# MiraPurkrabek/ProbPose_code

Measured on AMD Instinct MI355X. Metric: person-crops/sec @ 256x192 bs64, higher is better.
Workload: dtype f16x3; 1 GPU; ProbPose-small (ViT-S 12x384, 12 heads x 32) bs64 random 256x192 uint8 crops per GPU, flip_test=True, seeded random-init weights: preprocess -> backbone x2 passes -> ProbMapHead (heatmap branch + Sparsemax + 4 towers) -> ProbMap decode -> results in pinned host memory; crops_per_gpu=64, global_batch=64, parallelism=dp1, steps_in_flight=2

## Files before the change

probpose_code_amd/csrc/pp_api.hip:

```cpp
#include "pp_common.h"

#include <cstring>
#include <mutex>

namespace pp {

static thread_local char g_last_error[512] = "";

void set_error(const char* fmt, ...) {
    va_list ap;
    va_start(ap, fmt);
    vsnprintf(g_last_error, sizeof(g_last_error), fmt, ap);
    va_end(ap);
}

struct Option { const char* name; int value; };
static Option g_options[] = {
    {"panel", 1},
    {"conv_halo", 1},
    {"psplit_nst", 0},
    {"panel_linear_mink", 0},
    {"psplit_bf16_conv", 0},
    {"psplit_tap_inner", 1},
    {"psplit_conv_weight_major", 1},
    {"attn_dma", 1},
    {"conv_pool_split", 1},
    {"decode_wgs_per_cu", 3},
    {"linear_dma", 1},
    {"linear_loop", 1},
    {"psplit_deconv_weight_major", 0},
    {"ffn_pair", 1},
    {"psplit_tail", 1},
    {"wino_order", 8},
    {"ksplit_channels", 1},
    {"qkv_attn_deep", 1},
    {"skinny_tile", 0},
    {"qkv_attn_qsplit", 1},
    {"skinny_xcd_order", 1},
    {"ksplit9_below", 1024},
};

struct LaunchCount {
    char name[48];
    long long n;
};
static LaunchCount g_launches[96];
static int g_n_launches = 0;
static std::mutex g_launch_mutex;

void count_launch(const char* file_or_tag) {
    std::lock_guard<std::mutex> lock(g_launch_mutex);
    const char* base = file_or_tag;
    for (const char* c = file_or_tag; *c; ++c)
        if (*c == '/') base = c + 1;
    for (int i = 0; i < g_n_launches; ++i)
        if (std::strcmp(g_launches[i].name, base) == 0) {
            ++g_launches[i].n;
            return;
        }
    if (g_n_launches < (int)(sizeof(g_launches) / sizeof(g_launches[0]))) {
        std::snprintf(g_launches[g_n_launches].name, sizeof(g_launches[0].name), "%s", base);
        g_launches[g_n_launches++].n = 1;
    }
}

int option(const char* name) {
    for (const Option& o : g_options)
        if (std::strcmp(o.name, name) == 0) return o.value;
    return 0;
}

__global__ void clock_probe_kernel(unsigned long long* out, const unsigned long long* stop, unsigned long long ticks) {
    if (threadIdx.x != 0) return;
    const unsigned long long r0 = __builtin_amdgcn_s_memrealtime();
    const unsigned long long c0 = __builtin_amdgcn_s_memtime();
    unsigned long long r1 = r0;
    for (long long guard = 0; guard < (1ll << 21) && r1 - r0 < ticks; ++guard) {
        if (stop && __hip_atomic_load(stop, __ATOMIC_RELAXED, __HIP_MEMORY_SCOPE_SYSTEM) != 0) break;
        __builtin_amdgcn_s_sleep(127);
        r1 = __builtin_amdgcn_s_memrealtime();
    }
    const unsigned long long c1 = __builtin_amdgcn_s_memtime();
    r1 = __builtin_amdgcn_s_memrealtime();
    __hip_atomic_store(out + 0, c1 - c0, __ATOMIC_RELAXED, __HIP_MEMORY_SCOPE_SYSTEM);
    __hip_atomic_store(out + 1, r1 - r0, __ATOMIC_RELAXED, __HIP_MEMORY_SCOPE_SYSTEM);
}

}

extern "C" {

int pp_set_option(const char* name, int value) {
    using namespace pp;
    PP_REQUIRE(name, PP_ERR_INVALID_ARG, "pp_set_option: NULL name");
    for (Option& o : g_options)
        if (std::strcmp(o.name, name) == 0) {
            o.value = value;
            return PP_OK;
        }
    set_error("pp_set_option: unknown option '%s'", name);
    return PP_ERR_INVALID_ARG;
}

int pp_get_option(const char* name, int* value) {
    using namespace pp;
    PP_REQUIRE(name && value, PP_ERR_INVALID_ARG, "pp_get_option: NULL argument");
    for (const Option& o : g_options)
        if (std::strcmp(o.name, name) == 0) {
            *value = o.value;
            return PP_OK;
        }
    set_error("pp_get_option: unknown option '%s'", name);
    return PP_ERR_INVALID_ARG;
}

long long pp_launch_count(const char* kernel) {
    using namespace pp;
    if (!kernel) {
        set_error("pp_launch_count: NULL name");
        return 0;
    }
    std::lock_guard<std::mutex> lock(g_launch_mutex);
    for (int i = 0; i < g_n_launches; ++i)
        if (std::strcmp(g_launches[i].name, kernel) == 0) return g_launches[i].n;
    return 0;
}

int pp_reset_launch_counts(void) {
    std::lock_guard<std::mutex> lock(pp::g_launch_mutex);
    pp::g_n_launches = 0;
    return PP_OK;
}

long long pp_workspace_bytes(int buffer, int index, const pp_plan_shape* sh) {
    using namespace pp;
    if (!sh || sh->n_img <= 0 || sh->n_tokens <= 0 || sh->embed <= 0 || sh->ffn <= 0 || sh->n_keypoints <= 0 || sh->feat_h <= 0 || sh->feat_w <= 0 ||
        (sh->prec != PP_PREC_BF16 && sh->prec != PP_PREC_F32 && sh->prec != PP_PREC_F16X3)) {
        set_error("pp_workspace_bytes: bad plan shape");
        return PP_ERR_INVALID_ARG;
    }
    const long long esz = sh->prec == PP_PREC_BF16 ? 2 : 4;
    const long long M = (long long)sh->n_img * sh->n_tokens, E = sh->embed;
    auto tower_hw = [&](int j, long long& h, long long& w, long long& ph, long long& pw) {
        h = sh->feat_h;
        w = sh->feat_w;
        for (int i = 0;; ++i) {
            ph = i == 0 ? 4 : 2;
            pw = i == 0 ? 3 : 2;
            if (i == j) return;
            h /= ph;
            w /= pw;
        }
    };
    switch (buffer) {
        case PP_WS_PATCHES: return M * sh->patch_k * esz;
        case PP_WS_X: return M * E * 4;
        case PP_WS_H: case PP_WS_FEAT: case PP_WS_ATT: case PP_WS_LN2: return M * E * esz;
        case PP_WS_QKV: return M * 3 * E * esz;
        case PP_WS_FFN: return M * (long long)sh->ffn * esz;
        case PP_WS_LOGITS: return (long long)sh->n_img * sh->n_keypoints * sh->heat_h * sh->heat_w * 4;
        case PP_WS_DECONV: {
            if (index < 0 || index >= 8 || sh->deconv_channels <= 0) break;
            const long long up = 2ll << index;
            return (long long)sh->n_img * sh->feat_h * up * sh->feat_w * up * sh->deconv_channels * esz;
        }
        case PP_WS_TOWER: case PP_WS_TOWER_PARTIAL: case PP_WS_TOWER_POOLED: {
            if (index < 0 || index > 2) break;
            long long h, w, ph, pw;
            tower_hw(index, h, w, ph, pw);
            if (buffer == PP_WS_TOWER) return 4ll * sh->n_img * h * w * E * esz;
            if (buffer == PP_WS_TOWER_PARTIAL)
                return (long long)pp_conv3x3_splitk_slices(sh->prec, sh->n_img, (int)h, (int)w, sh->embed, sh->embed, 4) * 4 * sh->n_img * h * w * E * 4;
            return 4ll * sh->n_img * (h / ph) * (w / pw) * E * esz;
        }
        case PP_WS_LN_STATS: return E % 96 == 0 ? M * (E / 96) * 8 : 0;
        case PP_WS_WINOGRAD: {
            const long long n = pp_winograd_scratch_bytes(sh->n_img, sh->feat_h, sh->feat_w, sh->embed);
            return n > 0 ? n : 0;
        }
        default: break;
    }
    set_error("pp_workspace_bytes: unknown buffer %d (index %d)", buffer, index);
    return PP_ERR_INVALID_ARG;
}
// ... 58 lines not shown
```

probpose_code_amd/csrc/pp_ffn_dma.hip:

```cpp
#include "pp_common.h"
#include "pp_device.h"
#include "pp_split.h"
#include "pp_ffn_params.h"

namespace pp {
namespace ffd {

using ffs::Params;

constexpr int BM = 96, E = 384, CHUNK = 128;
constexpr int CW = 8, WAVES = 12, THREADS = WAVES * 64;
constexpr int KB = E / 32;
constexpr int G_KB = BM * 128;
constexpr int OFF_G = 0;
constexpr int OFF_RING = 4 * G_KB;
constexpr int SLOTB = 28 * 1024, NSLOT = 4;
constexpr int LDS = OFF_RING + NSLOT * SLOTB;
constexpr int X_OFF = 16 * 1024;
constexpr int NA = KB, NB = 8, STEPS = NA + NB;
constexpr int A_BLOCK = CHUNK * 128;
constexpr int B_BLOCK = (E / 2) * 128;
constexpr int B_PART = NA * A_BLOCK;
constexpr int CHUNK_BYTES = B_PART + NB * B_BLOCK;
constexpr int NPROJ = 2 * KB;
// ... 39 lines not shown

template <bool PROJ, bool PAIR>
__device__ __forceinline__ void dma_role(const Params& p, char* smem, int d, int lane, int m0, int nchunks, int c_rot) {
    char* const ring = smem + OFF_RING;
    const int x_l = lane >> 3;
    const unsigned v_w = (unsigned)lane * 16u;
    const unsigned v_x = (unsigned)(m0 + x_l) * (unsigned)(E * 4) + (unsigned)(((lane & 7) ^ x_l) << 4);

    if constexpr (PROJ) {
        auto issue_p = [&](int s) {
            if (s >= NPROJ) return;
            const __amdgpu_buffer_rsrc_t rw = buffer_rsrc(p.wproj, p.wproj_bytes);
#pragma unroll
            for (int u = 0; u < 6; ++u) {
                const int q = d + 4 * u;
                dma16(rw, ring + (s & 3) * SLOTB + q * 1024, v_w, s * B_BLOCK + q * 1024);
            }
            if ((s & 1) == 0) {
                const int kb = s >> 1;
                const __amdgpu_buffer_rsrc_t ra = buffer_rsrc(p.att, p.att_bytes);
#pragma unroll
                for (int u = 0; u < 3; ++u) {
                    const int q = d + 4 * u;
                    dma16(ra, smem + OFF_G + (kb & 3) * G_KB + q * 1024, v_x, kb * 128 + q * 8 * E * 4);
                }
            }
        };
        issue_p(0);
        issue_p(1);
        issue_p(2);
#pragma unroll
        for (int s = 0; s < NPROJ; ++s) {
            __builtin_amdgcn_sched_barrier(0);
            wait_vm_n(n_proj(s + 1) + n_proj(s + 2));
            __builtin_amdgcn_s_barrier();
            __builtin_amdgcn_sched_barrier(0);
            issue_p(s + 3);
        }
        __builtin_amdgcn_s_barrier();
        __builtin_amdgcn_s_barrier();
        __builtin_amdgcn_s_barrier();
        __builtin_amdgcn_s_barrier();
    }

    auto issue = [&](int ci, int t) {
        const bool live = ci < nchunks;
        int c = (live ? ci : 0) + c_rot;
        c = c >= nchunks ? c - nchunks : c;
        const int base = c * CHUNK_BYTES;
        const __amdgpu_buffer_rsrc_t rw = buffer_rsrc(p.wpack, live ? p.w_bytes : 0u);
        char* dst = ring + (t & 3) * SLOTB;
        if (t < NA) {
            const int kb = (ci & 1) ? NA - 1 - t : t;
#pragma unroll
            for (int u = 0; u < 4; ++u) {
                const int q = d + 4 * u;
                dma16(rw, dst + q * 1024, v_w, base + kb * A_BLOCK + q * 1024);
            }
            const __amdgpu_buffer_rsrc_t rh = buffer_rsrc(p.h, live ? p.h_bytes : 0u);
#pragma unroll
            for (int u = 0; u < 3; ++u) {
                const int q = d + 4 * u;
                dma16(rh, dst + X_OFF + q * 1024, v_x, kb * 128 + q * 8 * E * 4);
            }
        } else {
            const int sb = t - NA;
#pragma unroll
            for (int u = 0; u < 6; ++u) {
                const int q = d + 4 * u;
                dma16(rw, dst + q * 1024, v_w, base + B_PART + sb * B_BLOCK + q * 1024);
            }
        }
    };
    if constexpr (PAIR) {
        const int npairs = nchunks >> 1;
        auto issue2 = [&](int cp_, int t) {
            int cp = cp_;
            asm volatile("" : "+s"(cp));
            const bool live = cp < npairs;
            const int cpl = live ? cp : 0;
            const __amdgpu_buffer_rsrc_t rw = buffer_rsrc(p.wpack, live ? p.w_bytes : 0u);
            char* dst = ring + (t & 3) * SLOTB;
            if (t < 2 * NA) {
                int c = 2 * cpl + (t & 1) + c_rot;
                c = c >= nchunks ? c - nchunks : c;
                const int kb = (cp & 1) ? NA - 1 - (t >> 1) : (t >> 1);
#pragma unroll
                for (int u = 0; u < 4; ++u) {
                    const int q = d + 4 * u;
                    dma16(rw, dst + q * 1024, v_w, c * CHUNK_BYTES + kb * A_BLOCK + q * 1024);
                }
                if ((t & 1) == 0) {
                    const __amdgpu_buffer_rsrc_t rh = buffer_rsrc(p.h, live ? p.h_bytes : 0u);
#pragma unroll
                    for (int u = 0; u < 3; ++u) {
                        const int q = d + 4 * u;
                        dma16(rh, dst + X_OFF + q * 1024, v_x, kb * 128 + q * 8 * E * 4);
                    }
                }
            } else {
                const int which = (t - 2 * NA) >> 3, sb = (t - 2 * NA) & 7;
                int c = 2 * cpl + which + c_rot;
                c = c >= nchunks ? c - nchunks : c;
#pragma unroll
                for (int u = 0; u < 6; ++u) {
                    const int q = d + 4 * u;
                    dma16(rw, dst + q * 1024, v_w, c * CHUNK_BYTES + B_PART + sb * B_BLOCK + q * 1024);
                }
            }
        };
        constexpr int PS = 2 * STEPS;
        auto n2 = [](int t) { t %= PS; return t < 2 * NA ? ((t & 1) == 0 ? 7 : 4) : 6; };
        issue2(0, 0);
        issue2(0, 1);
        issue2(0, 2);
        for (int cp = 0; cp < npairs; ++cp) {
#pragma unroll
            for (int t = 0; t < PS; ++t) {
                __builtin_amdgcn_sched_barrier(0);
                wait_vm_n(n2(t + 1) + n2(t + 2));
                __builtin_amdgcn_s_barrier();
                __builtin_amdgcn_sched_barrier(0);
                if (t + 3 < PS) issue2(cp, t + 3); else issue2(cp + 1, t + 3 - PS);
                if (t == 2 * NA || t == 2 * NA + NB) __builtin_amdgcn_s_barrier();
            }
        }
    } else {
    issue(0, 0);
    issue(0, 1);
    issue(0, 2);
    for (int ci = 0; ci < nchunks; ++ci) {
#pragma unroll
        for (int t = 0; t < STEPS; ++t) {
            __builtin_amdgcn_sched_barrier(0);
            wait_vm_n(n_main(t + 1) + n_main(t + 2));
            __builtin_amdgcn_s_barrier();
            __builtin_amdgcn_sched_barrier(0);
            if (t + 3 < STEPS) issue(ci, t + 3); else issue(ci + 1, t + 3 - STEPS);
            if (t == NA) __builtin_amdgcn_s_barrier();
        }
    }
    }
    wait_vm<0>();
    __builtin_amdgcn_s_barrier();
    __builtin_amdgcn_s_barrier();
    __builtin_amdgcn_s_barrier();
}

#if FFD_STAMP
__device__ unsigned long long g_ffd_stamps[2][64];
#endif
struct TagF { static constexpr bool value = false; };
struct TagT { static constexpr bool value = true; };
template <bool PROJ, bool PAIR, int FOLD = 0>
__device__ __forceinline__ void compute_role(const Params& p, char* smem, int wv, int lane, int m0, int nchunks, int c_rot) {
    const int rg = wv >> 2, cg = wv & 3;
    const int f_row = lane & 15, f_kg = lane >> 4;
    auto chunk_of = [&](int i) { const int c = i + c_rot; return c >= nchunks ? c - nchunks : c; };
#if FFD_STAMP
    int n_stamp = 0;
    auto stamp = [&]() {
        if (wv == 0 && (blockIdx.x == 0 || blockIdx.x == 131)) {
            const unsigned long long t = __builtin_amdgcn_s_memtime();
            if (lane == 0 && n_stamp < 64) g_ffd_stamps[blockIdx.x == 0 ? 0 : 1][n_stamp] = t;
            ++n_stamp;
        }
    };
#else
    auto stamp = []() {};
#endif
    stamp();

    const int sw = f_row & 7;
    const int lane_hi = f_row * 128 + ((f_kg ^ sw) << 4), lane_lo = f_row * 128 + (((4 + f_kg) ^ sw) << 4);
    const int rows0 = rg * 48 + f_row;
    auto opaque_s = [](int v) { asm volatile("" : "+s"(v)); return v; };
    auto rd = [&](int lane_off, int uni, int imm) -> u32x4 { return *reinterpret_cast<const u32x4*>(smem + (lane_off + uni) + imm); };
    const int u_a = OFF_RING + cg * 32 * 128;
    const int u_b = OFF_RING + cg * 48 * 128;
    const int u_x = OFF_RING + X_OFF + rg * 48 * 128;
    const int u_g = OFF_G + rg * 48 * 128;

    f32x4 acc[3][6];
    f32x4 pacc[3][2];
    f32x4 b1v[2];
    u32x4 bgh[3], bgl[3];

    auto step_barrier = [&]() {
        __builtin_amdgcn_sched_barrier(0);
        wait_vm_lgkm<63>();
        __builtin_amdgcn_s_barrier();
        __builtin_amdgcn_sched_barrier(0);
    };
    auto b_step = [&](int slot, int half, int gbuf, bool load_g) {
        u32x4 wh[3], wl[3];
        const int ub = opaque_s(u_b + slot * SLOTB);
        const int ug = opaque_s(u_g + gbuf * G_KB);
        wh[0] = rd(lane_hi, ub, 0);
        if (load_g) bgh[0] = rd(lane_hi, ug, 0);
        wh[1] = rd(lane_hi, ub, 2048);
        wh[2] = rd(lane_hi, ub, 4096);
        if (load_g) {
            bgh[1] = rd(lane_hi, ug, 2048);
            bgh[2] = rd(lane_hi, ug, 4096);
        }
#pragma unroll
        for (int nf = 0; nf < 3; ++nf) wl[nf] = rd(lane_lo, ub, nf * 2048);
        if (load_g) {
#pragma unroll
            for (int rf = 0; rf < 3; ++rf) bgl[rf] = rd(lane_lo, ug, rf * 2048);
        }
        __builtin_amdgcn_sched_barrier(0);
#pragma unroll
        for (int rf = 0; rf < 3; ++rf)
#pragma unroll
            for (int nf = 0; nf < 3; ++nf) acc[rf][half * 3 + nf] = mma_f16(wh[nf], bgh[rf], acc[rf][half * 3 + nf]);
        __builtin_amdgcn_sched_barrier(0);
#pragma unroll
        for (int rf = 0; rf < 3; ++rf)
#pragma unroll
            for (int nf = 0; nf < 3; ++nf) acc[rf][half * 3 + nf] = mma_f16(wl[nf], bgh[rf], acc[rf][half * 3 + nf]);
        __builtin_amdgcn_sched_barrier(0);
#pragma unroll
        for (int nf = 0; nf < 3; ++nf)
#pragma unroll
            for (int rf = 0; rf < 3; ++rf) acc[rf][half * 3 + nf] = mma_f16(wh[nf], bgl[rf], acc[rf][half * 3 + nf]);
    };
    (void)b_step;
    auto layernorm_rows = [&](const float* gamma, const float* beta, float* x_dst, void* h_dst, bool store_x, auto fold_c) {
        constexpr bool FO = decltype(fold_c)::value;
        unsigned ones_ = ~0u;
        asm volatile("" : "+s"(ones_));
        const int ln_ = (int)__builtin_amdgcn_mbcnt_hi(ones_, __builtin_amdgcn_mbcnt_lo(ones_, 0u));
        const int fk_ = ln_ >> 4;
        const int rows0_ = rg * 48 + (ln_ & 15);
        auto shx = [&](float v, int m) -> float { return __builtin_bit_cast(float, __builtin_amdgcn_ds_bpermute((ln_ ^ m) << 2, __builtin_bit_cast(int, v))); };
        const unsigned row_ = (unsigned)(m0 + rows0_) * (unsigned)(E * 4);
        const unsigned v_rowx = row_ + (unsigned)fk_ * 16u;
        const unsigned v_rowh = row_ + (unsigned)fk_ * 8u;
        const unsigned v_rowh2 = row_ + (unsigned)(fk_ >> 1) * 16u + (unsigned)(fk_ & 1) * 64u;
        (void)v_rowh;
        const __amdgpu_buffer_rsrc_t rx = buffer_rsrc(x_dst, p.h_bytes);
        const __amdgpu_buffer_rsrc_t rh = buffer_rsrc(h_dst, p.h_bytes);
        float* stat = reinterpret_cast<float*>(smem + OFF_G);
        float mean[3], rstd[3];
#pragma unroll
        for (int rf = 0; rf < 3; ++rf) {
            float sm = 0.f;
#pragma unroll
            for (int cf = 0; cf < 6; ++cf) {
                const f32x4 v = acc[rf][cf];
                sm += (v[0] + v[1]) + (v[2] + v[3]);
            }
            sm += shx(sm, 16);
            sm += shx(sm, 32);
            if (fk_ == 0) stat[cg * BM + rows0_ + rf * 16] = sm;
        }
        __syncthreads();
#pragma unroll
        for (int rf = 0; rf < 3; ++rf) {
            const int r = rows0_ + rf * 16;
            mean[rf] = ((stat[r] + stat[BM + r]) + (stat[2 * BM + r] + stat[3 * BM + r])) * (1.0f / E);
            float q = 0.f;
#pragma unroll
            for (int cf = 0; cf < 6; ++cf)
#pragma unroll
                for (int k = 0; k < 4; ++k) {
                    const float dd = acc[rf][cf][k] - mean[rf];
                    q = __builtin_fmaf(dd, dd, q);
                }
            q += shx(q, 16);
            q += shx(q, 32);
            if (fk_ == 0) stat[(4 + cg) * BM + r] = q;
        }
        __syncthreads();
#if FFD_STAMP == 2
        stamp();
#endif
#pragma unroll
        for (int rf = 0; rf < 3; ++rf) {
            const int r = rows0_ + rf * 16;
            const float var = ((stat[4 * BM + r] + stat[5 * BM + r]) + (stat[6 * BM + r] + stat[7 * BM + r])) * (1.0f / E);
            rstd[rf] = 1.0f / sqrtf(var + p.eps);
            if (FO && fk_ == 0 && cg == 0 && m0 + r < p.M) {
                *reinterpret_cast<f32x2*>(p.stats_out + (size_t)(m0 + r) * 2) = f32x2{mean[rf], rstd[rf]};
            }
        }
        f32x4 gs_[6], bs_[6];
#pragma unroll
        for (int cf = 0; cf < 6; ++cf) {
            const int cb = (cf / 3) * 192 + cg * 48 + (cf % 3) * 16;
            gs_[cf] = FO ? f32x4{1.f, 1.f, 1.f, 1.f} : *reinterpret_cast<const f32x4*>(gamma + cb + fk_ * 4);
            bs_[cf] = FO ? f32x4{0.f, 0.f, 0.f, 0.f} : *reinterpret_cast<const f32x4*>(beta + cb + fk_ * 4);
        }
#pragma unroll
        for (int cf = 0; cf < 6; ++cf) {
            const int cb = (cf / 3) * 192 + cg * 48 + (cf % 3) * 16;
            const f32x4 g = gs_[cf], b = bs_[cf];
#pragma unroll
            for (int rf = 0; rf < 3; ++rf) {
                const f32x4 v = acc[rf][cf];
                float mu = mean[rf];
                const float rs = rstd[rf];
                asm("" : "+v"(mu));
                f32x4 hv = {(v[0] - mu) * rs * g[0] + b[0], (v[1] - mu) * rs * g[1] + b[1], (v[2] - mu) * rs * g[2] + b[2],
                            (v[3] - mu) * rs * g[3] + b[3]};
                if (FO) hv = f32x4{v[0] - mu, v[1] - mu, v[2] - mu, v[3] - mu};
#pragma unroll
                for (int j = 0; j < 4; ++j) { float t = hv[j]; split_pin(t); hv[j] = t; }
                if (store_x) {
                    const u32x4 vq = __builtin_bit_cast(u32x4, v);
                    store16_guarded(vq, rx, v_rowx + rf * (16 * E * 4), cb * 4);
                }
                u32x2 hu, lu;
                { unsigned h__, l__; split_pair(hv[0], hv[1], h__, l__); hu[0] = h__; lu[0] = l__; }
                { unsigned h__, l__; split_pair(hv[2], hv[3], h__, l__); hu[1] = h__; lu[1] = l__; }
                const int so = (cb >> 5) * 128 + (cb & 16) * 2;
                {
                    const auto s0 = __builtin_amdgcn_permlane16_swap(hu[0], lu[0], false, false);
                    const auto s1 = __builtin_amdgcn_permlane16_swap(hu[1], lu[1], false, false);
                    u32x4 q = {s0[0], s1[0], s0[1], s1[1]};
                    store16_guarded(q, rh, v_rowh2 + rf * (16 * E * 4), so);
                }
            }
        }
    };

    float res_mean[3] = {0.f, 0.f, 0.f};
    if constexpr ((FOLD & 1) != 0) {
#pragma unroll
        for (int rf = 0; rf < 3; ++rf) {
            const int r = m0 + rows0 + rf * 16;
            res_mean[rf] = r < p.M ? p.res_stats[(size_t)r * 2] : 0.f;
        }
    }
    const __amdgpu_buffer_rsrc_t rres = buffer_rsrc(p.residual, p.h_bytes);
    const unsigned v_rowx = (unsigned)(m0 + rows0) * (unsigned)(E * 4) + (unsigned)f_kg * 16u;
#pragma unroll
    for (int rf = 0; rf < 3; ++rf)
#pragma unroll
        for (int cf = 0; cf < 6; ++cf) {
            const int cb = (cf / 3) * 192 + cg * 48 + (cf % 3) * 16;
            if constexpr ((FOLD & 1) != 0) {
                const unsigned vsp = (unsigned)(m0 + rows0) * (unsigned)(E * 4) + (unsigned)(f_kg >> 1) * 16u + (unsigned)(f_kg & 1) * 64u;
                const u32x4 q = __builtin_bit_cast(u32x4, __builtin_amdgcn_raw_buffer_load_b128(rres, vsp + rf * (16 * E * 4), (cb >> 5) * 128 + (cb & 16) * 2, 0));
                const auto s0 = __builtin_amdgcn_permlane16_swap(q[0], q[2], false, false);
                const auto s1 = __builtin_amdgcn_permlane16_swap(q[1], q[3], false, false);
                const f16x4 hh = __builtin_bit_cast(f16x4, u32x2{s0[0], s1[0]}), ll = __builtin_bit_cast(f16x4, u32x2{s0[1], s1[1]});
                const float mu = res_mean[rf];
                acc[rf][cf] = f32x4{((float)hh[0] + (float)ll[0]) + mu, ((float)hh[1] + (float)ll[1]) + mu, ((float)hh[2] + (float)ll[2]) + mu,
                                    ((float)hh[3] + (float)ll[3]) + mu};
            } else {
                acc[rf][cf] = __builtin_bit_cast(f32x4, __builtin_amdgcn_raw_buffer_load_b128(rres, v_rowx + rf * (16 * E * 4), cb * 4, 0));
            }
        }

    stamp();
    {
        const float s_in = PROJ ? p.s_p : p.s_2;
#pragma unroll
        for (int cf = 0; cf < 6; ++cf) {
            f32x4 bv = {0.f, 0.f, 0.f, 0.f};
            if constexpr (!PROJ) bv = *reinterpret_cast<const f32x4*>(p.b2 + (cf / 3) * 192 + cg * 48 + (cf % 3) * 16 + f_kg * 4);
#pragma unroll
            for (int rf = 0; rf < 3; ++rf) acc[rf][cf] = (acc[rf][cf] + bv) * s_in;
        }
    }
    if constexpr (PROJ) {
        {
            u32x4 pwh[3], pwl[3];
            step_barrier();
            {
                const int ub = opaque_s(u_b), ug = opaque_s(u_g);
#pragma unroll
                for (int nf = 0; nf < 3; ++nf) { pwh[nf] = rd(lane_hi, ub, nf * 2048); pwl[nf] = rd(lane_lo, ub, nf * 2048); }
#pragma unroll
                for (int rf = 0; rf < 3; ++rf) { bgl[rf] = rd(lane_lo, ug, rf * 2048); bgh[rf] = rd(lane_hi, ug, rf * 2048); }
            }
#pragma unroll 1
            for (int kp = 0; kp < NPROJ / 4; ++kp) {
#pragma unroll
                for (int q = 0; q < 4; ++q) {
                    const int half = q & 1;
                    const int ub_n = opaque_s(u_b + ((q + 1) & 3) * SLOTB);
                    const int ug_n = opaque_s(u_g + ((((4 * kp + q) >> 1) + 1) & 3) * G_KB);
                    const bool nb = q < 3 || kp + 1 < NPROJ / 4;
                    const bool newg = nb && half == 1;
                    __builtin_amdgcn_sched_barrier(0);
#pragma unroll
                    for (int i = 0; i < 9; ++i) {
                        const int rf = i / 3, nf = i % 3;
                        acc[rf][half * 3 + nf] = mma_f16(pwh[nf], bgl[rf], acc[rf][half * 3 + nf]);
                        __builtin_amdgcn_sched_barrier(0);
                        if (i == 1 && nb) step_barrier();
                        if (nf == 2 && newg) bgl[rf] = rd(lane_lo, ug_n, rf * 2048);
                        __builtin_amdgcn_sched_barrier(0);
                    }
#pragma unroll
                    for (int i = 0; i < 9; ++i) {
                        const int rf = i / 3, nf = i % 3;
                        acc[rf][half * 3 + nf] = mma_f16(pwh[nf], bgh[rf], acc[rf][half * 3 + nf]);
                        __builtin_amdgcn_sched_barrier(0);
                        if (rf == 2 && nb) pwh[nf] = rd(lane_hi, ub_n, nf * 2048);
                        __builtin_amdgcn_sched_barrier(0);
                    }
#pragma unroll
                    for (int i = 0; i < 9; ++i) {
                        const int rf = i / 3, nf = i % 3;
                        acc[rf][half * 3 + nf] = mma_f16(pwl[nf], bgh[rf], acc[rf][half * 3 + nf]);
                        __builtin_amdgcn_sched_barrier(0);
                        if (nf == 2 && newg) bgh[rf] = rd(lane_hi, ug_n, rf * 2048);
                        if (rf == 2 && nb) pwl[nf] = rd(lane_lo, ub_n, nf * 2048);
                        __builtin_amdgcn_sched_barrier(0);
                    }
                }
            }
        }
#pragma unroll
        for (int cf = 0; cf < 6; ++cf) {
            const f32x4 bv = *reinterpret_cast<const f32x4*>(p.bp + (cf / 3) * 192 + cg * 48 + (cf % 3) * 16 + f_kg * 4);
#pragma unroll
            for (int rf = 0; rf < 3; ++rf) acc[rf][cf] = acc[rf][cf] * p.inv_p + bv;
        }
        stamp();
        __syncthreads();
#if FFD_STAMP == 2
        stamp();
#endif
        layernorm_rows(p.gamma2, p.beta2, nullptr, const_cast<void*>(p.h), false, TagF{});
#if FFD_STAMP == 2
        stamp();
#endif
        wait_vm_lgkm<0>();
#if FFD_STAMP == 2
        stamp();
#endif
        __syncthreads();
        stamp();
    }

    if constexpr (PROJ) {
#pragma unroll
        for (int cf = 0; cf < 6; ++cf) {
            const f32x4 bv = *reinterpret_cast<const f32x4*>(p.b2 + (cf / 3) * 192 + cg * 48 + (cf % 3) * 16 + f_kg * 4);
#pragma unroll
            for (int rf = 0; rf < 3; ++rf) acc[rf][cf] = (acc[rf][cf] + bv) * p.s_2;
        }
    }
    auto load_b1 = [&](int ci) {
        const int c = chunk_of(ci < nchunks ? ci : 0);
#pragma unroll
        for (int nf = 0; nf < 2; ++nf) b1v[nf] = *reinterpret_cast<const f32x4*>(p.b1 + c * CHUNK + cg * 32 + nf * 16 + f_kg * 4);
    };
    load_b1(0);

    auto gelu_chunk = [&](f32x4 (&pa)[3][2]) __attribute__((always_inline)) {
#pragma unroll
        for (int rf = 0; rf < 3; ++rf)
#pragma unroll
            for (int nf = 0; nf < 2; ++nf) {
                int ln_ = lane;
                asm volatile("" : "+v"(ln_));
                const int fk_ = ln_ >> 4, sw_ = ln_ & 7;
                char* gs = smem + OFF_G + cg * G_KB + (rg * 48 + (ln_ & 15) + rf * 16) * 128 + (fk_ & 1) * 8;
                const int c = 2 * nf + (fk_ >> 1);
                const int sw = sw_;
                unsigned hq[2], lq[2];
#pragma unroll
                for (int u0 = 0; u0 < 2; ++u0) {
                    const f32x2 x = f32x2{pa[rf][nf][2 * u0], pa[rf][nf][2 * u0 + 1]} * p.inv_1;
                    const f32x2 ax = __builtin_elementwise_abs(x);
                    const f32x2 d = ax * 0.23164189265f + 1.0f;
                    const f32x2 t = {__builtin_amdgcn_rcpf(d[0]), __builtin_amdgcn_rcpf(d[1])};
                    const f32x2 uu = x * 0.84932180028801904272f;
                    const f32x2 u2 = uu * uu;
                    const f32x2 e = {__builtin_amdgcn_exp2f(-u2[0]), __builtin_amdgcn_exp2f(-u2[1])};
                    f32x2 q = t * 1.061405429f + -1.453152027f;
                    q = t * q + 1.421413741f;
                    q = t * q + -0.284496736f;
                    q = t * q + 0.254829592f;
                    const f32x2 erfc_z = (t * q) * e;
                    const f32x2 ma = ax * -0.5f;
                    const f32x2 mx = x * 0.5f - ma;
                    f32x2 g = ma * erfc_z + mx;
                    asm("" : "+v"(g));
                    const f16x2 hp = __builtin_convertvector(g, f16x2);
                    const unsigned hu = __builtin_bit_cast(unsigned, hp);
                    f32x2 l;
                    asm("v_fma_mix_f32 %0, %1, 1.0, -%2 op_sel:[0,0,0] op_sel_hi:[0,0,1]" : "=v"(l[0]) : "v"(g[0]), "v"(hu));
                    asm("v_fma_mix_f32 %0, %1, 1.0, -%2 op_sel:[0,0,1] op_sel_hi:[0,0,1]" : "=v"(l[1]) : "v"(g[1]), "v"(hu));
                    hq[u0] = hu;
                    lq[u0] = __builtin_bit_cast(unsigned, __builtin_convertvector(l, f16x2));
                }
                *reinterpret_cast<u32x2*>(gs + ((c ^ sw) << 4)) = u32x2{hq[0], hq[1]};
                *reinterpret_cast<u32x2*>(gs + (((4 + c) ^ sw) << 4)) = u32x2{lq[0], lq[1]};
            }
    };

    if constexpr (PAIR) {
        f32x4 pacc1[3][2];
        u32x4 wh[2], wl[2], xh[3], xl[3], bwh[3], bwl[3];
        const __amdgpu_buffer_rsrc_t rb1 = buffer_rsrc(p.b1, (unsigned)p.F * 4u);
        auto load_b1x = [&](int ci, f32x4 (&dst)[2]) __attribute__((always_inline)) {
            const int c = chunk_of(ci < nchunks ? ci : 0);
            int vo = lane;
            asm volatile("" : "+v"(vo));
            vo &= 0x30;
#pragma unroll
            for (int nf = 0; nf < 2; ++nf) dst[nf] = __builtin_bit_cast(f32x4, __builtin_amdgcn_raw_buffer_load_b128(rb1, vo, (c * CHUNK + cg * 32 + nf * 16) * 4, 0));
        };
        f32x4 b1w[2];
        load_b1x(1, b1w);
        step_barrier();
        {
            const int ua = opaque_s(u_a), ux = opaque_s(u_x);
#pragma unroll
            for (int nf = 0; nf < 2; ++nf) { wh[nf] = rd(lane_hi, ua, nf * 2048); wl[nf] = rd(lane_lo, ua, nf * 2048); }
#pragma unroll
            for (int rf = 0; rf < 3; ++rf) { xl[rf] = rd(lane_lo, ux, rf * 2048); xh[rf] = rd(lane_hi, ux, rf * 2048); }
        }
        auto a_step = [&](f32x4 (&pa)[3][2], int slot_next, bool reload_x, bool to_b) __attribute__((always_inline)) {
            const int sn = (slot_next & 3) * SLOTB;
            const int ua_n = opaque_s(u_a + sn), ux_n = opaque_s(u_x + sn), ub_n = opaque_s(u_b + sn);
            __builtin_amdgcn_sched_barrier(0);
#pragma unroll
            for (int i = 0; i < 6; ++i) {
                const int rf = i >> 1, nf = i & 1;
                mma_ip(wh[nf], xl[rf], pa[rf][nf]);
                __builtin_amdgcn_sched_barrier(0);
                if (i == 1) step_barrier();
                if (reload_x && !to_b && nf == 1) xl[rf] = rd(lane_lo, ux_n, rf * 2048);
                __builtin_amdgcn_sched_barrier(0);
            }
#pragma unroll
            for (int i = 0; i < 6; ++i) {
                const int rf = i >> 1, nf = i & 1;
                mma_ip(wh[nf], xh[rf], pa[rf][nf]);
                __builtin_amdgcn_sched_barrier(0);
                if (rf == 2) { if (!to_b) wh[nf] = rd(lane_hi, ua_n, nf * 2048); else bwh[nf] = rd(lane_hi, ub_n, nf * 2048); }
                if (to_b && i == 5) bwh[2] = rd(lane_hi, ub_n, 2 * 2048);
                __builtin_amdgcn_sched_barrier(0);
            }
#pragma unroll
            for (int i = 0; i < 6; ++i) {
                const int rf = i >> 1, nf = i & 1;
                mma_ip(wl[nf], xh[rf], pa[rf][nf]);
                __builtin_amdgcn_sched_barrier(0);
                if (reload_x && !to_b && nf == 1) xh[rf] = rd(lane_hi, ux_n, rf * 2048);
                if (rf == 2) { if (!to_b) wl[nf] = rd(lane_lo, ua_n, nf * 2048); else bwl[nf] = rd(lane_lo, ub_n, nf * 2048); }
                if (to_b && i == 5) bwl[2] = rd(lane_lo, ub_n, 2 * 2048);
                __builtin_amdgcn_sched_barrier(0);
            }
        };
        auto b_phase = [&](int t0, int next, bool more) __attribute__((always_inline)) {
            {
                const int ug = opaque_s(u_g);
#pragma unroll
                for (int rf = 0; rf < 3; ++rf) { bgl[rf] = rd(lane_lo, ug, rf * 2048); bgh[rf] = rd(lane_hi, ug, rf * 2048); }
            }
            auto two_steps = [&](int jb, bool last_kb) __attribute__((always_inline)) {
#pragma unroll
                for (int half = 0; half < 2; ++half) {
                    const int sb = 2 * jb + half;
                    const int sn = ((t0 + sb + 1) & 3) * SLOTB;
                    const int ub_n = opaque_s(u_b + sn), ua_n = opaque_s(u_a + sn), ux_n = opaque_s(u_x + sn);
                    const int ug_n = opaque_s(u_g + ((jb + 1) & 3) * G_KB);
                    const bool nb = !(last_kb && half == 1);
                    const bool newg = nb && half == 1;
                    const bool wnext = nb || next == 0;
                    const bool anext = !nb && next == 1;
                    __builtin_amdgcn_sched_barrier(0);
#pragma unroll
                    for (int i = 0; i < 9; ++i) {
                        const int rf = i / 3, nf = i % 3;
                        mma_ip(bwh[nf], bgl[rf], acc[rf][half * 3 + nf]);
                        __builtin_amdgcn_sched_barrier(0);
                        if (i == 1 && (nb || next == 0 || more)) step_barrier();
                        if (nf == 2) { if (newg) bgl[rf] = rd(lane_lo, ug_n, rf * 2048); else if (anext) xl[rf] = rd(lane_lo, ux_n, rf * 2048); }
                        __builtin_amdgcn_sched_barrier(0);
                    }
#pragma unroll
                    for (int i = 0; i < 9; ++i) {
                        const int rf = i / 3, nf = i % 3;
                        mma_ip(bwh[nf], bgh[rf], acc[rf][half * 3 + nf]);
                        __builtin_amdgcn_sched_barrier(0);
                        if (rf == 2) { if (wnext) bwh[nf] = rd(lane_hi, ub_n, nf * 2048); else if (anext && nf < 2) wh[nf] = rd(lane_hi, ua_n, nf * 2048); }
                        __builtin_amdgcn_sched_barrier(0);
                    }
#pragma unroll
                    for (int i = 0; i < 9; ++i) {
                        const int rf = i / 3, nf = i % 3;
                        mma_ip(bwl[nf], bgh[rf], acc[rf][half * 3 + nf]);
                        __builtin_amdgcn_sched_barrier(0);
                        if (nf == 2) { if (newg) bgh[rf] = rd(lane_hi, ug_n, rf * 2048); else if (anext) xh[rf] = rd(lane_hi, ux_n, rf * 2048); }
                        if (rf == 2) { if (wnext) bwl[nf] = rd(lane_lo, ub_n, nf * 2048); else if (anext && nf < 2) wl[nf] = rd(lane_lo, ua_n, nf * 2048); }
                        __builtin_amdgcn_sched_barrier(0);
                    }
                }
            };
#pragma unroll 1
            for (int jb = 0; jb < NB / 2 - 1; ++jb) two_steps(jb, false);
            two_steps(NB / 2 - 1, true);
        };
        const int npairs = nchunks >> 1;
        for (int cp = 0; cp < npairs; ++cp) {
#pragma unroll
            for (int rf = 0; rf < 3; ++rf)
#pragma unroll
                for (int nf = 0; nf < 2; ++nf) { pacc[rf][nf] = b1v[nf] * p.s_1; pacc1[rf][nf] = b1w[nf] * p.s_1; }
            valu_settle(pacc);
            valu_settle(pacc1);
#pragma unroll 1
            for (int kbi = 0; kbi < NA - 1; ++kbi) {
                a_step(pacc, 2 * kbi + 1, false, false);
                a_step(pacc1, 2 * kbi + 2, true, false);
            }
            a_step(pacc, 2 * NA - 1, false, false);
            a_step(pacc1, 2 * NA, true, true);
            stamp();
            mfma_settle(pacc);
            gelu_chunk(pacc);
            step_barrier();
            stamp();
            load_b1x(2 * cp + 2, b1v);
            b_phase(2 * NA, 0, true);
            stamp();
            mfma_settle(pacc1);
            gelu_chunk(pacc1);
            step_barrier();
            stamp();
            load_b1x(2 * cp + 3, b1w);
            b_phase(2 * NA + NB, 1, cp + 1 < npairs);
            stamp();
        }
        mfma_settle(acc);
    } else {
    {
        u32x4 wh[2], wl[2], xh[3], xl[3];
        u32x4 bwh[3], bwl[3];
        step_barrier();
        {
            const int ua = opaque_s(u_a), ux = opaque_s(u_x);
#pragma unroll
            for (int nf = 0; nf < 2; ++nf) { wh[nf] = rd(lane_hi, ua, nf * 2048); wl[nf] = rd(lane_lo, ua, nf * 2048); }
#pragma unroll
            for (int rf = 0; rf < 3; ++rf) { xl[rf] = rd(lane_lo, ux, rf * 2048); xh[rf] = rd(lane_hi, ux, rf * 2048); }
        }
        for (int ci = 0; ci < nchunks; ++ci) {
#pragma unroll
            for (int rf = 0; rf < 3; ++rf)
#pragma unroll
                for (int nf = 0; nf < 2; ++nf) pacc[rf][nf] = b1v[nf] * p.s_1;
            load_b1(ci + 1);
#pragma unroll
            for (int t = 0; t < NA; ++t) {
                const int sn = ((t + 1) & 3) * SLOTB;
                const int ua_n = opaque_s(u_a + sn), ux_n = opaque_s(u_x + sn), ub_n = opaque_s(u_b + sn);
                const bool na = t + 1 < NA;
                __builtin_amdgcn_sched_barrier(0);
#pragma unroll
                for (int i = 0; i < 6; ++i) {
                    const int rf = i >> 1, nf = i & 1;
                    pacc[rf][nf] = mma_f16(wh[nf], xl[rf], pacc[rf][nf]);
                    __builtin_amdgcn_sched_barrier(0);
                    if (i == 1) step_barrier();
                    if (na && nf == 1) xl[rf] = rd(lane_lo, ux_n, rf * 2048);
                    __builtin_amdgcn_sched_barrier(0);
                }
#pragma unroll
                for (int i = 0; i < 6; ++i) {
                    const int rf = i >> 1, nf = i & 1;
                    pacc[rf][nf] = mma_f16(wh[nf], xh[rf], pacc[rf][nf]);
                    __builtin_amdgcn_sched_barrier(0);
                    if (rf == 2) { if (na) wh[nf] = rd(lane_hi, ua_n, nf * 2048); else bwh[nf] = rd(lane_hi, ub_n, nf * 2048); }
                    if (!na && i == 5) bwh[2] = rd(lane_hi, ub_n, 2 * 2048);
                    __builtin_amdgcn_sched_barrier(0);
                }
#pragma unroll
                for (int i = 0; i < 6; ++i) {
                    const int rf = i >> 1, nf = i & 1;
                    pacc[rf][nf] = mma_f16(wl[nf], xh[rf], pacc[rf][nf]);
                    __builtin_amdgcn_sched_barrier(0);
                    if (na && nf == 1) xh[rf] = rd(lane_hi, ux_n, rf * 2048);
                    if (rf == 2) { if (na) wl[nf] = rd(lane_lo, ua_n, nf * 2048); else bwl[nf] = rd(lane_lo, ub_n, nf * 2048); }
                    if (!na && i == 5) bwl[2] = rd(lane_lo, ub_n, 2 * 2048);
                    __builtin_amdgcn_sched_barrier(0);
                }
            }
            gelu_chunk(pacc);
            step_barrier();
            {
                const int ug = opaque_s(u_g);
#pragma unroll
                for (int rf = 0; rf < 3; ++rf) { bgl[rf] = rd(lane_lo, ug, rf * 2048); bgh[rf] = rd(lane_hi, ug, rf * 2048); }
            }
#pragma unroll
            for (int sb = 0; sb < NB; ++sb) {
                const int half = sb & 1;
                const int sn = ((NA + sb + 1) & 3) * SLOTB;
                const int ub_n = opaque_s(u_b + sn), ua_n = opaque_s(u_a + sn), ux_n = opaque_s(u_x + sn);
                const int ug_n = opaque_s(u_g + (((sb >> 1) + 1) & 3) * G_KB);
                const bool nb = sb + 1 < NB;
                const bool newg = nb && half == 1;
                __builtin_amdgcn_sched_barrier(0);
#pragma unroll
                for (int i = 0; i < 9; ++i) {
                    const int rf = i / 3, nf = i % 3;
                    acc[rf][half * 3 + nf] = mma_f16(bwh[nf], bgl[rf], acc[rf][half * 3 + nf]);
                    __builtin_amdgcn_sched_barrier(0);
                    if (i == 1 && (nb || ci + 1 < nchunks)) step_barrier();
                    if (nf == 2) { if (newg) bgl[rf] = rd(lane_lo, ug_n, rf * 2048); else if (!nb) xl[rf] = rd(lane_lo, ux_n, rf * 2048); }
                    __builtin_amdgcn_sched_barrier(0);
                }
#pragma unroll
                for (int i = 0; i < 9; ++i) {
                    const int rf = i / 3, nf = i % 3;
                    acc[rf][half * 3 + nf] = mma_f16(bwh[nf], bgh[rf], acc[rf][half * 3 + nf]);
                    __builtin_amdgcn_sched_barrier(0);
                    if (rf == 2) { if (nb) bwh[nf] = rd(lane_hi, ub_n, nf * 2048); else if (nf < 2) wh[nf] = rd(lane_hi, ua_n, nf * 2048); }
                    __builtin_amdgcn_sched_barrier(0);
                }
#pragma unroll
                for (int i = 0; i < 9; ++i) {
                    const int rf = i / 3, nf = i % 3;
                    acc[rf][half * 3 + nf] = mma_f16(bwl[nf], bgh[rf], acc[rf][half * 3 + nf]);
                    __builtin_amdgcn_sched_barrier(0);
                    if (nf == 2) { if (newg) bgh[rf] = rd(lane_hi, ug_n, rf * 2048); else if (!nb) xh[rf] = rd(lane_hi, ux_n, rf * 2048); }
                    if (rf == 2) { if (nb) bwl[nf] = rd(lane_lo, ub_n, nf * 2048); else if (nf < 2) wl[nf] = rd(lane_lo, ua_n, nf * 2048); }
                    __builtin_amdgcn_sched_barrier(0);
                }
            }
        }
    }
    }
    __syncthreads();
    stamp();
#pragma unroll
    for (int rf = 0; rf < 3; ++rf)
#pragma unroll
        for (int cf = 0; cf < 6; ++cf) acc[rf][cf] *= p.inv_2;
    if constexpr ((FOLD & 2) != 0) layernorm_rows(nullptr, nullptr, nullptr, p.h_out, false, TagT{});
    else layernorm_rows(p.gamma, p.beta, p.x_out, p.h_out, true, TagF{});
    stamp();
}

template <bool PROJ, bool PAIR, int FOLD = 0>
__device__ __forceinline__ void body(const Params p) {
    extern __shared__ __attribute__((aligned(16))) char smem[];
    const int tid = threadIdx.x, lane = tid & 63;
    const int wv = __builtin_amdgcn_readfirstlane(tid >> 6);
    const int m0 = blockIdx.x * BM;
    const int nchunks = p.F / CHUNK;
    const int c_rot = (int)(blockIdx.x & 7) % nchunks;
    if (wv >= CW) dma_role<PROJ, PAIR>(p, smem, wv - CW, lane, m0, nchunks, c_rot);
    else compute_role<PROJ, PAIR, FOLD>(p, smem, wv, lane, m0, nchunks, c_rot);
}

__global__ __launch_bounds__(THREADS) void ffn_dma_kernel(const Params p) { body<false, false>(p); }
__global__ __launch_bounds__(THREADS) void proj_ffn_dma_kernel(const Params p) { body<true, false>(p); }
__global__ __launch_bounds__(THREADS) void ffn_dma_pair_kernel(const Params p) { body<false, true>(p); }
__global__ __launch_bounds__(THREADS) void proj_ffn_dma_pair_kernel(const Params p) { body<true, true>(p); }
__global__ __launch_bounds__(THREADS) void proj_ffn_dma_pair_fold1_kernel(const Params p) { body<true, true, 1>(p); }
__global__ __launch_bounds__(THREADS) void proj_ffn_dma_pair_fold2_kernel(const Params p) { body<true, true, 2>(p); }
__global__ __launch_bounds__(THREADS) void proj_ffn_dma_pair_fold3_kernel(const Params p) { body<true, true, 3>(p); }

}

#if FFD_STAMP
extern "C" int pp_dev_ffd_stamps(unsigned long long* out) {
    return (int)hipMemcpyFromSymbol(out, HIP_SYMBOL(pp::ffd::g_ffd_stamps), sizeof(unsigned long long) * 128, 0, hipMemcpyDeviceToHost);
}
#endif

namespace ffs {
int launch_dma_form(const Params& p, bool proj, hipStream_t s) {
    const bool pair = option("ffn_pair") != 0 && (p.F / ffd::CHUNK) % 2 == 0;
    auto kern = pair ? (proj ? ffd::proj_ffn_dma_pair_kernel : ffd::ffn_dma_pair_kernel) : (proj ? ffd::proj_ffn_dma_kernel : ffd::ffn_dma_kernel);
    const int fold = (p.res_split ? 1 : 0) | (p.fold_out ? 2 : 0);
    if (fold) {
        kern = fold == 1 ? ffd::proj_ffn_dma_pair_fold1_kernel : fold == 2 ? ffd::proj_ffn_dma_pair_fold2_kernel : ffd::proj_ffn_dma_pair_fold3_kernel;
    }
    PP_HIP_CHECK(hipFuncSetAttribute(reinterpret_cast<const void*>(kern), hipFuncAttributeMaxDynamicSharedMemorySize, ffd::LDS));
    hipLaunchKernelGGL(kern, dim3((p.M + ffd::BM - 1) / ffd::BM), dim3(ffd::THREADS), ffd::LDS, s, p);
    PP_LAUNCH_CHECK_AS(fold ? "ffn_dma_fold" : pair ? "ffn_dma_pair" : "ffn_dma_single");
    return PP_OK;
}
}
}
```

Baseline: 14710 crops/s.

## Interleave GELU of second FFN chunk into MFMA gaps of B phase

Adds a GFILL variant of the paired FFN DMA kernel that computes the GELU (erf polynomial, exp, f16 hi/lo split) for most of the second up-projection chunk. This is done op-by-op with inline asm between the down-projection MFMAs of the preceding B phase. The goal is to hide the VALU GELU work under matrix-core latency instead of running it serially after the phase. gelu_chunk then skips the already-converted fragments. The B-phase loop is fully unrolled in the fill path, which grows code size and register pressure. An option selects between fill and nofill kernel variants, with fill enabled by default.

```diff
diff --git a/probpose_code_amd/csrc/pp_api.hip b/probpose_code_amd/csrc/pp_api.hip
--- a/probpose_code_amd/csrc/pp_api.hip
+++ b/probpose_code_amd/csrc/pp_api.hip
@@ -30,6 +30,7 @@
     {"linear_loop", 1},
     {"psplit_deconv_weight_major", 0},
     {"ffn_pair", 1},
+    {"ffn_gelu_fill", 1},
     {"psplit_tail", 1},
     {"wino_order", 8},
     {"ksplit_channels", 1},
diff --git a/probpose_code_amd/csrc/pp_ffn_dma.hip b/probpose_code_amd/csrc/pp_ffn_dma.hip
--- a/probpose_code_amd/csrc/pp_ffn_dma.hip
+++ b/probpose_code_amd/csrc/pp_ffn_dma.hip
@@ -215,7 +215,7 @@
 #endif
 struct TagF { static constexpr bool value = false; };
 struct TagT { static constexpr bool value = true; };
-template <bool PROJ, bool PAIR, int FOLD = 0>
+template <bool PROJ, bool PAIR, int FOLD = 0, bool GFILL = false>
 __device__ __forceinline__ void compute_role(const Params& p, char* smem, int wv, int lane, int m0, int nchunks, int c_rot) {
     const int rg = wv >> 2, cg = wv & 3;
     const int f_row = lane & 15, f_kg = lane >> 4;
@@ -517,7 +517,7 @@
     };
     load_b1(0);
 
-    auto gelu_chunk = [&](f32x4 (&pa)[3][2]) __attribute__((always_inline)) {
+    auto gelu_chunk = [&](f32x4 (&pa)[3][2], int done) __attribute__((always_inline)) {
 #pragma unroll
         for (int rf = 0; rf < 3; ++rf)
 #pragma unroll
@@ -529,6 +529,10 @@
                 const int c = 2 * nf + (fk_ >> 1);
                 const int sw = sw_;
                 unsigned hq[2], lq[2];
+                if (rf * 2 + nf < done) {
+                    const u32x4 w = __builtin_bit_cast(u32x4, pa[rf][nf]);
+                    hq[0] = w[0]; hq[1] = w[1]; lq[0] = w[2]; lq[1] = w[3];
+                } else
 #pragma unroll
                 for (int u0 = 0; u0 < 2; ++u0) {
                     const f32x2 x = f32x2{pa[rf][nf][2 * u0], pa[rf][nf][2 * u0 + 1]} * p.inv_1;
@@ -615,15 +619,68 @@
                 __builtin_amdgcn_sched_barrier(0);
             }
         };
-        auto b_phase = [&](int t0, int next, bool more) __attribute__((always_inline)) {
+        float gt[2], gq[2];
+        auto fill_gap = [&](int G) __attribute__((always_inline)) {
+            constexpr int OPS = 20;
+            if (G < 0 || G >= 10 * OPS) return;
+            const int P = G / OPS, op = G % OPS, k = 2 * (P & 1);
+            f32x4& v = pacc1[P >> 2][(P >> 1) & 1];
+            auto one = [&](int i) __attribute__((always_inline)) {
+                float x = v[k + i];
+                switch (op) {
+                    case 0: asm volatile("v_mul_f32 %0, %1, %2" : "=v"(x) : "s"(p.inv_1), "v"(v[k + i])); break;
+                    case 1: asm volatile("v_fma_f32 %0, |%1|, %2, 1.0" : "=v"(gt[i]) : "v"(x), "s"(0.23164189265f)); break;
+                    case 2: if (i == 0) asm volatile("v_rcp_f32 %0, %0" : "+v"(gt[0])); break;
+                    case 3: if (i == 0) asm volatile("v_rcp_f32 %0, %0" : "+v"(gt[1])); break;
+                    case 4: asm volatile("v_mov_b32 %0, %1" : "=v"(gq[i]) : "s"(-1.453152027f)); break;
+                    case 5: asm volatile("v_fmac_f32 %0, %1, %2" : "+v"(gq[i]) : "s"(1.061405429f), "v"(gt[i])); break;
+                    case 6: asm volatile("v_fma_f32 %0, %1, %0, %2" : "+v"(gq[i]) : "v"(gt[i]), "s"(1.421413741f)); break;
+                    case 7: asm volatile("v_fma_f32 %0, %1, %0, %2" : "+v"(gq[i]) : "v"(gt[i]), "s"(-0.284496736f)); break;
+                    case 8: asm volatile("v_fma_f32 %0, %1, %0, %2" : "+v"(gq[i]) : "v"(gt[i]), "s"(0.254829592f)); break;
+                    case 9: asm volatile("v_mul_f32 %0, %1, %0" : "+v"(gq[i]) : "v"(gt[i])); break;
+                    case 10: asm volatile("v_mul_f32 %0, %1, %2" : "=v"(gt[i]) : "s"(0.84932180028801904272f), "v"(x)); break;
+                    case 11: asm volatile("v_mul_f32 %0, %0, %0" : "+v"(gt[i])); break;
+                    case 12: if (i == 0) asm volatile("v_exp_f32 %0, -%0" : "+v"(gt[0])); break;
+                    case 13: if (i == 0) asm volatile("v_exp_f32 %0, -%0" : "+v"(gt[1])); break;
+                    case 14: asm volatile("v_mul_f32 %0, %1, %0" : "+v"(gq[i]) : "v"(gt[i])); break;
+                    case 15: asm volatile("v_mul_f32_e64 %0, |%1|, -0.5" : "=v"(gt[i]) : "v"(x)); break;
+                    case 16: asm volatile("v_fma_f32 %0, %0, 0.5, -%1" : "+v"(x) : "v"(gt[i])); break;
+                    case 17: asm volatile("v_fma_f32 %0, %1, %2, %0" : "+v"(x) : "v"(gt[i]), "v"(gq[i])); break;
+                    case 18:
+                        if (i == 0) {
+                            asm volatile("v_cvt_pk_f16_f32 %0, %1, %2" : "=v"(gq[0]) : "v"(v[k]), "v"(v[k + 1]));
+                            asm volatile("v_fma_mix_f32 %0, %1, 1.0, -%2 op_sel:[0,0,0] op_sel_hi:[0,0,1]" : "=v"(gt[0]) : "v"(v[k]), "v"(gq[0]));
+                        }
+                        break;
+                    default:
+                        if (i == 0) {
+                            asm volatile("v_fma_mix_f32 %0, %1, 1.0, -%2 op_sel:[0,0,1] op_sel_hi:[0,0,1]" : "=v"(gt[1]) : "v"(v[k + 1]), "v"(gq[0]));
+                            asm volatile("v_cvt_pk_f16_f32 %0, %1, %2" : "=v"(gq[1]) : "v"(gt[0]), "v"(gt[1]));
+                        }
+                        break;
+                }
+                if (op == 0 || op == 16 || op == 17) v[k + i] = x;
+            };
+            one(0);
+            one(1);
+            if (op == 19) {
+                if (k == 0) { v[0] = gq[0]; v[1] = gq[1]; }
+                else {
+                    v[2] = v[1]; v[1] = gq[0]; v[3] = gq[1];
+                    asm volatile("" : "+v"(v));
+                }
+            }
+        };
+        (void)fill_gap;
+        auto b_phase = [&](int t0, int next, bool more, bool fill) __attribute__((always_inline)) {
+            if (fill) mfma_settle(pacc1);
             {
                 const int ug = opaque_s(u_g);
 #pragma unroll
                 for (int rf = 0; rf < 3; ++rf) { bgl[rf] = rd(lane_lo, ug, rf * 2048); bgh[rf] = rd(lane_hi, ug, rf * 2048); }
             }
-            auto two_steps = [&](int jb, bool last_kb) __attribute__((always_inline)) {
-#pragma unroll
-                for (int half = 0; half < 2; ++half) {
+            auto one_step = [&](int jb, int half, bool last_kb) __attribute__((always_inline)) {
+                {
                     const int sb = 2 * jb + half;
                     const int sn = ((t0 + sb + 1) & 3) * SLOTB;
                     const int ub_n = opaque_s(u_b + sn), ua_n = opaque_s(u_a + sn), ux_n = opaque_s(u_x + sn);
@@ -638,6 +695,7 @@
                         const int rf = i / 3, nf = i % 3;
                         mma_ip(bwh[nf], bgl[rf], acc[rf][half * 3 + nf]);
                         __builtin_amdgcn_sched_barrier(0);
+                        if (fill && i >= 2) fill_gap(sb * 25 + i - 2);
                         if (i == 1 && (nb || next == 0 || more)) step_barrier();
                         if (nf == 2) { if (newg) bgl[rf] = rd(lane_lo, ug_n, rf * 2048); else if (anext) xl[rf] = rd(lane_lo, ux_n, rf * 2048); }
                         __builtin_amdgcn_sched_barrier(0);
@@ -647,6 +705,7 @@
                         const int rf = i / 3, nf = i % 3;
                         mma_ip(bwh[nf], bgh[rf], acc[rf][half * 3 + nf]);
                         __builtin_amdgcn_sched_barrier(0);
+                        if (fill) fill_gap(sb * 25 + 7 + i);
                         if (rf == 2) { if (wnext) bwh[nf] = rd(lane_hi, ub_n, nf * 2048); else if (anext && nf < 2) wh[nf] = rd(lane_hi, ua_n, nf * 2048); }
                         __builtin_amdgcn_sched_barrier(0);
                     }
@@ -655,14 +714,25 @@
                         const int rf = i / 3, nf = i % 3;
                         mma_ip(bwl[nf], bgh[rf], acc[rf][half * 3 + nf]);
                         __builtin_amdgcn_sched_barrier(0);
+                        if (fill) fill_gap(sb * 25 + 16 + i);
                         if (nf == 2) { if (newg) bgh[rf] = rd(lane_hi, ug_n, rf * 2048); else if (anext) xh[rf] = rd(lane_hi, ux_n, rf * 2048); }
                         if (rf == 2) { if (wnext) bwl[nf] = rd(lane_lo, ub_n, nf * 2048); else if (anext && nf < 2) wl[nf] = rd(lane_lo, ua_n, nf * 2048); }
                         __builtin_amdgcn_sched_barrier(0);
                     }
                 }
             };
+            auto two_steps = [&](int jb, bool last_kb) __attribute__((always_inline)) {
+                one_step(jb, 0, last_kb);
+                one_step(jb, 1, last_kb);
+            };
+            if (fill) {
+                two_steps(0, false);
+                two_steps(1, false);
+                two_steps(2, false);
+            } else {
 #pragma unroll 1
-            for (int jb = 0; jb < NB / 2 - 1; ++jb) two_steps(jb, false);
+                for (int jb = 0; jb < NB / 2 - 1; ++jb) two_steps(jb, false);
+            }
             two_steps(NB / 2 - 1, true);
         };
         const int npairs = nchunks >> 1;
@@ -682,18 +752,19 @@
             a_step(pacc1, 2 * NA, true, true);
             stamp();
             mfma_settle(pacc);
-            gelu_chunk(pacc);
+            gelu_chunk(pacc, 0);
             step_barrier();
             stamp();
-            load_b1x(2 * cp + 2, b1v);
-            b_phase(2 * NA, 0, true);
+            if (!GFILL) load_b1x(2 * cp + 2, b1v);
+            b_phase(2 * NA, 0, true, GFILL);
             stamp();
-            mfma_settle(pacc1);
-            gelu_chunk(pacc1);
+            if (!GFILL) mfma_settle(pacc1);
+            gelu_chunk(pacc1, GFILL ? 5 : 0);
             step_barrier();
             stamp();
+            if (GFILL) load_b1x(2 * cp + 2, b1v);
             load_b1x(2 * cp + 3, b1w);
-            b_phase(2 * NA + NB, 1, cp + 1 < npairs);
+            b_phase(2 * NA + NB, 1, cp + 1 < npairs, false);
             stamp();
         }
         mfma_settle(acc);
@@ -750,7 +821,7 @@
                     __builtin_amdgcn_sched_barrier(0);
                 }
             }
-            gelu_chunk(pacc);
+            gelu_chunk(pacc, 0);
             step_barrier();
             {
                 const int ug = opaque_s(u_g);
@@ -807,7 +878,7 @@
     stamp();
 }
 
-template <bool PROJ, bool PAIR, int FOLD = 0>
+template <bool PROJ, bool PAIR, int FOLD = 0, bool GFILL = false>
 __device__ __forceinline__ void body(const Params p) {
     extern __shared__ __attribute__((aligned(16))) char smem[];
     const int tid = threadIdx.x, lane = tid & 63;
@@ -816,16 +887,21 @@
     const int nchunks = p.F / CHUNK;
     const int c_rot = (int)(blockIdx.x & 7) % nchunks;
     if (wv >= CW) dma_role<PROJ, PAIR>(p, smem, wv - CW, lane, m0, nchunks, c_rot);
-    else compute_role<PROJ, PAIR, FOLD>(p, smem, wv, lane, m0, nchunks, c_rot);
+    else compute_role<PROJ, PAIR, FOLD, GFILL>(p, smem, wv, lane, m0, nchunks, c_rot);
 }
 
 __global__ __launch_bounds__(THREADS) void ffn_dma_kernel(const Params p) { body<false, false>(p); }
 __global__ __launch_bounds__(THREADS) void proj_ffn_dma_kernel(const Params p) { body<true, false>(p); }
-__global__ __launch_bounds__(THREADS) void ffn_dma_pair_kernel(const Params p) { body<false, true>(p); }
-__global__ __launch_bounds__(THREADS) void proj_ffn_dma_pair_kernel(const Params p) { body<true, true>(p); }
-__global__ __launch_bounds__(THREADS) void proj_ffn_dma_pair_fold1_kernel(const Params p) { body<true, true, 1>(p); }
-__global__ __launch_bounds__(THREADS) void proj_ffn_dma_pair_fold2_kernel(const Params p) { body<true, true, 2>(p); }
-__global__ __launch_bounds__(THREADS) void proj_ffn_dma_pair_fold3_kernel(const Params p) { body<true, true, 3>(p); }
+__global__ __launch_bounds__(THREADS) void ffn_dma_pair_kernel(const Params p) { body<false, true, 0, true>(p); }
+__global__ __launch_bounds__(THREADS) void proj_ffn_dma_pair_kernel(const Params p) { body<true, true, 0, true>(p); }
+__global__ __launch_bounds__(THREADS) void proj_ffn_dma_pair_fold1_kernel(const Params p) { body<true, true, 1, true>(p); }
+__global__ __launch_bounds__(THREADS) void proj_ffn_dma_pair_fold2_kernel(const Params p) { body<true, true, 2, true>(p); }
+__global__ __launch_bounds__(THREADS) void proj_ffn_dma_pair_fold3_kernel(const Params p) { body<true, true, 3, true>(p); }
+__global__ __launch_bounds__(THREADS) void ffn_dma_pair_nofill_kernel(const Params p) { body<false, true>(p); }
+__global__ __launch_bounds__(THREADS) void proj_ffn_dma_pair_nofill_kernel(const Params p) { body<true, true>(p); }
+__global__ __launch_bounds__(THREADS) void proj_ffn_dma_pair_fold1_nofill_kernel(const Params p) { body<true, true, 1>(p); }
+__global__ __launch_bounds__(THREADS) void proj_ffn_dma_pair_fold2_nofill_kernel(const Params p) { body<true, true, 2>(p); }
+__global__ __launch_bounds__(THREADS) void proj_ffn_dma_pair_fold3_nofill_kernel(const Params p) { body<true, true, 3>(p); }
 
 }
 
@@ -838,10 +914,14 @@
 namespace ffs {
 int launch_dma_form(const Params& p, bool proj, hipStream_t s) {
     const bool pair = option("ffn_pair") != 0 && (p.F / ffd::CHUNK) % 2 == 0;
-    auto kern = pair ? (proj ? ffd::proj_ffn_dma_pair_kernel : ffd::ffn_dma_pair_kernel) : (proj ? ffd::proj_ffn_dma_kernel : ffd::ffn_dma_kernel);
+    const bool gfill = option("ffn_gelu_fill") != 0;
+    auto kern = pair ? (proj ? (gfill ? ffd::proj_ffn_dma_pair_kernel : ffd::proj_ffn_dma_pair_nofill_kernel) : (gfill ? ffd::ffn_dma_pair_kernel : ffd::ffn_dma_pair_nofill_kernel))
+                     : (proj ? ffd::proj_ffn_dma_kernel : ffd::ffn_dma_kernel);
     const int fold = (p.res_split ? 1 : 0) | (p.fold_out ? 2 : 0);
     if (fold) {
-        kern = fold == 1 ? ffd::proj_ffn_dma_pair_fold1_kernel : fold == 2 ? ffd::proj_ffn_dma_pair_fold2_kernel : ffd::proj_ffn_dma_pair_fold3_kernel;
+        kern = fold == 1 ? (gfill ? ffd::proj_ffn_dma_pair_fold1_kernel : ffd::proj_ffn_dma_pair_fold1_nofill_kernel)
+               : fold == 2 ? (gfill ? ffd::proj_ffn_dma_pair_fold2_kernel : ffd::proj_ffn_dma_pair_fold2_nofill_kernel)
+                           : (gfill ? ffd::proj_ffn_dma_pair_fold3_kernel : ffd::proj_ffn_dma_pair_fold3_nofill_kernel);
     }
     PP_HIP_CHECK(hipFuncSetAttribute(reinterpret_cast<const void*>(kern), hipFuncAttributeMaxDynamicSharedMemorySize, ffd::LDS));
     hipLaunchKernelGGL(kern, dim3((p.M + ffd::BM - 1) / ffd::BM), dim3(ffd::THREADS), ffd::LDS, s, p);
```

Result: no change. 14770 crops/s (median of 6 runs) (+0.4%).
